# HorizonRobotics/HoloAgent

Hardware: AMD Instinct MI355X
Metric: HMSG frames/sec (one scene per GPU: map A1-A2, fusion A3-A5, merge A6, pooling A7, floors A8, rooms by the device watershed N1, room clouds, room embeddings and View nodes A9, objects with the view <-> object test A10 and graph assembly A11, nothing handed in -- plus 1000 coarse-to-fine retrieval qu (higher is better)
Workload: dtype f64 geometry / f32 features

## Files before the change

holoagent_amd/_lib.py:

```python
from __future__ import annotations

import ctypes as C
import os

import numpy as np

_HERE = os.path.dirname(os.path.abspath(__file__))
LIB_PATH = os.path.join(_HERE, "libhmsg.so")


class HmsgConfig(C.Structure):
    _fields_ = [
        ("device_id", C.c_int32), ("feat_dim", C.c_int32), ("height", C.c_int32), ("width", C.c_int32),
        ("max_frames", C.c_int32), ("max_masks", C.c_int32),
        ("voxel_size", C.c_double), ("depth_scale", C.c_double), ("init_overlap_thresh", C.c_double),
        ("overlap_thresh_factor", C.c_double), ("iou_thresh", C.c_double), ("clip_masked_weight", C.c_double),
        ("max_mask_distance", C.c_double), ("merge_type", C.c_int32), ("outlier_nb_points", C.c_int32),
        ("outlier_radius", C.c_double), ("pool_max_dist", C.c_double), ("feat_dbscan_eps", C.c_double),
        ("feat_dbscan_min", C.c_int32), ("merge_dbscan_eps", C.c_double), ("merge_dbscan_min", C.c_int32),
        ("min_instance_points", C.c_int32), ("skip_frames", C.c_int32), ("depth_cut", C.c_double), ("grid_resolution", C.c_double),
        ("overlap_distance_form", C.c_int32),
    ]


# ... 168 lines not shown
    "hmsg_test_allocator_carving": (C.c_int, [C.c_int32, C.c_int32]),
    "hmsg_test_dbscan": (C.c_int, [_P, C.c_int32, _P, C.c_double, C.c_int32, _P, _P, _P, _P, _P]),
    "hmsg_index_load_objects": (C.c_int, [C.c_int32, C.c_char_p, C.c_int64, _P, _P, C.c_int32, C.POINTER(_P), C.POINTER(C.c_int32)]),
    "hmsg_index_create": (C.c_int, [C.c_int32, C.c_int32, C.c_int64, _P, C.c_int32, _P, C.POINTER(_P)]),
    "hmsg_index_destroy": (None, [_P]),
    "hmsg_index_last_error": (C.c_char_p, [_P]),
    "hmsg_index_set_profiling": (C.c_int, [_P, C.c_int32]),
    "hmsg_index_profile": (C.c_int, [_P, C.POINTER(C.c_int64), C.POINTER(C.c_double), C.POINTER(C.c_double)]),
    "hmsg_query_objects": (C.c_int, [_P, C.c_int32, C.c_int32, _P, _P, _P, _P, C.c_int32, C.c_int32, _P, _P, _P]),
    "hmsg_similarity": (C.c_int, [_P, C.c_int32, _P, _P]),
    "hmsg_index_set_hierarchy": (C.c_int, [_P, C.c_int32, C.c_int32, _P, _P, _P, _P, _P, _P]),
    "hmsg_query_hier": (C.c_int, [_P, C.c_int32, C.c_int32, _P, _P, _P, _P, _P, C.c_int32, C.c_int32, C.c_int32, _P, _P, _P, _P, _P]),
    "hmsg_comm_unique_id": (C.c_int, [_P]),
    "hmsg_comm_create": (C.c_int, [_P, C.c_int32, C.c_int32, C.c_int32, C.POINTER(_P)]),
    "hmsg_comm_destroy": (None, [_P]),
    "hmsg_comm_last_error": (C.c_char_p, [_P]),
    "hmsg_allgather_nodes": (C.c_int, [_P, _P, C.c_int32, C.POINTER(_P), _P, _P]),
    "hmsg_allreduce_feature_sums": (C.c_int, [_P, _P]),
    "hmsg_test_sort_pairs": (C.c_int, [_P, _P, C.c_int64, C.c_int32]),
    "hmsg_test_repeat_add": (C.c_int, [_P, _P, _P, _P, C.c_int64]),
    "hmsg_test_ckdtree": (C.c_int, [_P, C.c_int64, _P, C.c_int64, _P, _P, _P]),
    "hmsg_test_boundary": (C.c_int, [C.c_int32, _P, C.c_int64]),
    "hmsg_test_group_pairs": (C.c_int, [C.c_int32, C.c_int64, _P, C.c_int32, _P, C.c_double, _P, C.c_int64, C.POINTER(C.c_int64)]),
    "hmsg_test_pool_rows": (C.c_int, [C.c_int32, C.c_int32, _P, _P, _P, _P, C.c_int64, C.c_int32, C.c_double, C.c_int32, _P]),
}
EXPORTED_SYMBOLS = tuple(_SIGS)


class HmsgLib:
    def __init__(self, path: str | None = None):
        path = path or LIB_PATH
        if not os.path.exists(path):
            raise HmsgError(
                f"{path} not found: build the HIP library first (python -c 'import __graft_entry__ as g; g.build()' "
                "or make -C holoagent_amd/csrc).  There is no CPU fallback.")
        self.path = path
        self.c = C.CDLL(path)
        for name, (res, args) in _SIGS.items():
            fn = getattr(self.c, name)
            fn.restype = res
            fn.argtypes = args
        if self.c.hmsg_config_size() != C.sizeof(HmsgConfig):
            raise HmsgError("struct hmsg_config of %s has %d bytes, the binding's HmsgConfig %d: rebuild the library or update "
                            "holoagent_amd/_lib.py" % (path, self.c.hmsg_config_size(), C.sizeof(HmsgConfig)))

    def default_config(self, **over) -> HmsgConfig:
# ... 1207 lines not shown
```

holoagent_amd/csrc/hmsg_merge.hip:

```cpp
#include "hmsg_boundary.h"
#include "hmsg_cloudops.h"
#include "hmsg_fold_host.h"

#include <algorithm>
#include <cmath>
#include <numeric>
#include <chrono>
#include <unordered_map>
#include <condition_variable>
#include <deque>
#include <mutex>
#include <thread>

namespace {

struct Cloud {
    long long off = 0;
    int n = 0;
    double mn[3] = {0, 0, 0}, mx[3] = {0, 0, 0};
    bool fixed = false;
    bool fresh = true;
    bool raw = false;
    bool anchor = false;
    unsigned long long uid = 0;
// ... 91 lines not shown
                           long long cursor_base, int chunk) {
    const OvGrid g = gr[find_entry(gr, ngr, blockIdx.x)];
    const int i0 = (int)(blockIdx.x - (unsigned)g.blk0) * chunk, i1 = min(g.n, i0 + chunk);
    for (int i = i0 + threadIdx.x; i < i1; i += blockDim.x) {
        const double* p = pool + (size_t)(g.pt_off + i) * 3;
        atomicAdd(&cursor[ov_cell(g, (float)p[0], (float)p[1], (float)p[2]) - cursor_base], 1u);
    }
}
__global__ void k_ov_fill(const double* __restrict__ pool, const OvGrid* __restrict__ gr, int ngr, const unsigned* __restrict__ cells,
                          unsigned* __restrict__ cursor, long long cursor_base, float* __restrict__ sorted, int chunk) {
    const OvGrid g = gr[find_entry(gr, ngr, blockIdx.x)];
    const int i0 = (int)(blockIdx.x - (unsigned)g.blk0) * chunk, i1 = min(g.n, i0 + chunk);
    for (int i = i0 + threadIdx.x; i < i1; i += blockDim.x) {
        const double* p = pool + (size_t)(g.pt_off + i) * 3;
        float x = (float)p[0], y = (float)p[1], z = (float)p[2];
        long long c = ov_cell(g, x, y, z);
        size_t pos = (size_t)g.ix_pt + cells[c] + (atomicSub(&cursor[c - cursor_base], 1u) - 1u);
        sorted[(size_t)pos * 3] = x;
        sorted[(size_t)pos * 3 + 1] = y;
        sorted[(size_t)pos * 3 + 2] = z;
    }
}

#define OV_UNROLL 4
__device__ __forceinline__ float ov_norm2(float a, float b, float c) { return __fadd_rn(__fadd_rn(__fmul_rn(a, a), __fmul_rn(b, b)), __fmul_rn(c, c)); }
template <bool BLAS>
__device__ __forceinline__ float ov_dist2(float x, float y, float z, float qx, float qy, float qz, float nx) {
    if (!BLAS) {
        const float ddx = __fsub_rn(x, qx), ddy = __fsub_rn(y, qy), ddz = __fsub_rn(z, qz);
        return __fadd_rn(__fadd_rn(__fmul_rn(ddx, ddx), __fmul_rn(ddy, ddy)), __fmul_rn(ddz, ddz));
    }
    const float ip = __fmaf_rn(z, qz, __fmaf_rn(y, qy, __fmul_rn(x, qx)));
    const float d = __fsub_rn(__fadd_rn(nx, ov_norm2(qx, qy, qz)), __fmul_rn(2.0f, ip));
    return d < 0.f ? 0.f : d;
}
template <bool BLAS = false>
__device__ __forceinline__ bool ov_scan(const float* __restrict__ sorted, unsigned s0, unsigned e0, float x, float y, float z,
                                        float r2, unsigned* ncand = nullptr, float nx = 0.f) {
    for (unsigned k = s0; k < e0; k += OV_UNROLL) {
        bool h = false;
#pragma unroll
        for (int j = 0; j < OV_UNROLL; ++j) {
            const unsigned kk = min(k + (unsigned)j, e0 - 1u);
            const float d2 = ov_dist2<BLAS>(x, y, z, sorted[(size_t)kk * 3], sorted[(size_t)kk * 3 + 1], sorted[(size_t)kk * 3 + 2], nx);
            h = h || (k + (unsigned)j < e0 && d2 < r2);
        }
// ... 376 lines not shown
            hipLaunchKernelGGL(k_gp_pairs<true>, dim3((unsigned)tiles.size()), dim3(GP_TILE), 0, s, d_box, d_tiles, iou_thresh, n,
                               (unsigned*)nullptr, (const unsigned*)start.p, h_out.p, cap);
            HMSG_CHECK_LAUNCH();
            spin.wait(s);
            const long long total = (long long)(unsigned)h_out.p[0];
            if (total <= cap) {
                *n_pairs = total;
                return h_out.p + 2;
            }
            cap_pairs = total;
            h_out.ensure(2 + 2 * (size_t)cap_pairs);
        }
    }
    static bool fits(const int* group_off, int n_groups) {
        unsigned long long worst = 0;
        for (int g = 0; g < n_groups; ++g) {
            const unsigned long long m = (unsigned long long)(group_off[g + 1] - group_off[g]);
            worst += m * (m ? m - 1 : 0) / 2;
        }
        return worst < (1ull << 32);
    }
};

double bbox_iou(const Cloud& a, const Cloud& b) {
    return box_iou(a.mn, a.mx, b.mn, b.mx);
}

struct IntSpan {
    const int* b;
    const int* e;
    size_t size() const { return (size_t)(e - b); }
    int operator[](size_t k) const { return b[k]; }
    const int* begin() const { return b; }
    const int* end() const { return e; }
};
struct CompList {
    std::vector<int> off, mem;
    size_t size() const { return off.empty() ? 0 : off.size() - 1; }
    IntSpan operator[](size_t c) const { return IntSpan{mem.data() + off[c], mem.data() + off[c + 1]}; }
};

struct Merger {
    hmsg_ctx* h = nullptr;
    hipStream_t s = nullptr;
    CloudOps ops;
    DevBuf<double> pool;
// ... 1 lines not shown
    long long pool_used = 0;
    DevBuf<unsigned> ix_cells;
    long long ix_cells_used = 0;
    DevBuf<float> ix_pts;
    long long ix_pts_used = 0;
    DevBuf<double> concat;
    DevBuf<unsigned char> concat_core;
    DevBuf<OvGrid> d_grids;
    PinnedBuf<OvGrid> h_grids;
    PinnedBuf<CatSeg> h_cat;
    DevBuf<unsigned> d_cursor;
    DevBuf<CatSeg> d_cat;
    DevBuf<unsigned long long> ovstat;
    Publisher pub_counts;
    PinnedBuf<char> h_ovpack;
    DevBuf<char> d_ovpack;
    PinnedBuf<OvSpec> h_spec[2];
    DevBuf<OvGrid> d_spec[2];
    int spec_turn = 0;
    std::vector<OvSpec> spec;
    std::vector<int> spec_of_seg;
    bool spec_wanted = getenv("HMSG_DEBUG_NO_SPEC_INDEX") == nullptr;
    double spec_built = 0, spec_built_pts = 0, spec_skipped = 0;
    size_t cursor_clean = 0;
    SpinWait spin;
    unsigned long long next_uid = 1;
    std::unordered_map<unsigned long long, double> ratio_cache;
    bool use_cache = false;
    bool use_anchor = true;
    bool inplace_wanted = getenv("HMSG_DEBUG_NO_INPLACE") == nullptr;
    double radius = 0;
    double reach = 0;
    int faiss_form = 0;
    double cell = 0;
    double eps = 0.1;
    int minpts = 10;
    double iou_thresh = 0.05;
    double tphase[6] = {0, 0, 0, 0, 0, 0};
    struct Stats {
        double steps = 0, clouds = 0, fresh_raw = 0, fresh_g = 0, pairs_raw = 0, pairs_g = 0;
        double scan1_raw = 0, scan2_raw = 0, scan1_g = 0, scan2_g = 0;
        double idx_pts = 0;
        double ccount[5] = {0, 0, 0, 0, 0}, cpts[5] = {0, 0, 0, 0, 0}, cB[5] = {0, 0, 0, 0, 0}, cmem[5] = {0, 0, 0, 0, 0};
        double cchanged[5] = {0, 0, 0, 0, 0}, cmulti[5] = {0, 0, 0, 0, 0}, ccontested[5] = {0, 0, 0, 0, 0}, cnonfixed[5] = {0, 0, 0, 0, 0};
    } st;
    bool want_stats = false;

    template <typename T>
    void grow(DevBuf<T>& b, size_t used_elems, size_t need_elems) {
        if (need_elems <= b.n) return;
        CarveScope carve;
        DevBuf<T> nb;
        nb.alloc(std::max(need_elems * 2, (size_t)1 << 18));
        if (used_elems) HIP_TRY(hipMemcpyAsync(nb.p, b.p, used_elems * sizeof(T), hipMemcpyDeviceToDevice, s));
        HIP_TRY(hipStreamSynchronize(s));
        nb.swap(b);
    }

    OvGrid grid_at(const Cloud& c, const float* lo, const int* gd, long long ix_cell, long long ix_pt, long long pt_off, int n) const {
        OvGrid g;
        g.blk0 = 0;
        g.next = -1;
        g.pt_off = pt_off;
        g.ix_cell = ix_cell;
        g.ix_pt = ix_pt;
        g.n = n;
        g.gx = gd[0];
        g.gy = gd[1];
        g.gz = gd[2];
        g.mnx = (float)c.mn[0]; g.mny = (float)c.mn[1]; g.mnz = (float)c.mn[2];
        g.mxx = (float)c.mx[0]; g.mxy = (float)c.mx[1]; g.mxz = (float)c.mx[2];
        g.ox = (double)lo[0] - 1e-3;
        g.oy = (double)lo[1] - 1e-3;
        g.oz = (double)lo[2] - 1e-3;
        g.cell = cell;
        return g;
    }
    void push_grids(const Cloud& c, std::vector<OvGrid>& g) const {
        g.push_back(grid_at(c, c.bmn, c.gd, c.ix_cell, c.ix_pt, c.off, c.n));
        g.back().blk0 = c.nb;
        if (c.has_delta) {
            g.back().next = (int)g.size();
            g.push_back(grid_at(c, c.dmn, c.gd2, c.ix_cell2, c.ix_pt2, c.off + c.nb, c.n - c.nb));
        }
    }

    void build_indices(std::vector<Cloud>& L) {
        std::vector<int> todo;
        long long ncell_new = 0, npts_new = 0;
        int maxn = 0;
        std::vector<OvGrid> g;
        unsigned nblk = 0;
        for (int i = 0; i < (int)L.size(); ++i) {
            Cloud& c = L[i];
            if (c.has_index || c.n == 0) continue;
            const float lo[3] = {(float)c.mn[0], (float)c.mn[1], (float)c.mn[2]};
            int gd[3];
            for (int a = 0; a < 3; ++a) gd[a] = (int)std::floor(((double)(float)c.mx[a] - (double)lo[a] + 2e-3) / cell) + 1;
            const long long ncell = (long long)gd[0] * gd[1] * gd[2] + 1;
// ... 165 lines not shown
                sp.delta_always = delta_always ? 1 : 0;
                sp.out_off = sd.out_mode ? sd.out_off : out_base;
                sp.ncell = ncell;
                spec_of_seg[(size_t)sg] = (int)spec.size();
                spec.push_back(sp);
                nblk += cdiv((size_t)sd.n, OVI_CHUNK);
                ncell_new += ncell;
                npts_max += sd.n;
            }
        if (spec.empty()) return;
        if (!(ncell_new < (1ll << 31) && npts_max < (1ll << 31))) {
            spec.clear();
            spec_of_seg.assign(segs.size(), -1);
            return;
        }
        grow(ix_cells, (size_t)ix_cells_used, (size_t)(ix_cells_used + ncell_new));
        grow(ix_pts, (size_t)ix_pts_used * 3, (size_t)(ix_pts_used + npts_max) * 3);
        spec_turn ^= 1;
        PinnedBuf<OvSpec>& hs = h_spec[spec_turn];
        DevBuf<OvGrid>& ds = d_spec[spec_turn];
        hs.ensure(spec.size());
        ds.ensure(spec.size());
        memcpy(hs.p, spec.data(), spec.size() * sizeof(OvSpec));
        hipLaunchKernelGGL(k_ov_spec, dim3(cdiv(spec.size(), 64)), dim3(64), 0, s, (const OvSpec*)hs.p, (int)spec.size(), d_res, K, ds.p);
        {
            const unsigned* before = d_cursor.p;
            d_cursor.ensure((size_t)ncell_new);
            if (d_cursor.p != before) cursor_clean = 0;
            if (cursor_clean < (size_t)ncell_new) {
                HIP_TRY(hipMemsetAsync(d_cursor.p, 0, d_cursor.n * 4, s));
                cursor_clean = d_cursor.n;
            }
        }
        hipLaunchKernelGGL(k_ov_count, dim3(nblk), dim3(256), 0, s, (const double*)pool.p, (const OvGrid*)ds.p, (int)spec.size(),
                           d_cursor.p, ix_cells_used, OVI_CHUNK);
        HMSG_CHECK_LAUNCH();
        hmsg_scan_u32(d_cursor.p, ix_cells.p + ix_cells_used, (size_t)ncell_new, s, ops.scan_tmp, nullptr);
        hipLaunchKernelGGL(k_ov_fill, dim3(nblk), dim3(256), 0, s, (const double*)pool.p, (const OvGrid*)ds.p, (int)spec.size(),
                           (const unsigned*)ix_cells.p, d_cursor.p, ix_cells_used, ix_pts.p, OVI_CHUNK);
        HMSG_CHECK_LAUNCH();
    }

    void overlap_ratios(const std::vector<Cloud>& L, const std::vector<std::pair<int, int>>& pairs, std::vector<double>& ratio,
                        double decide_th, std::vector<unsigned char>* second_ran = nullptr) {
        ratio.assign(pairs.size(), 0.0);
        if (second_ran) second_ran->assign(pairs.size(), 0);
        if (pairs.empty()) return;
        const size_t P = pairs.size();
        const auto pack_t0 = std::chrono::steady_clock::now();
        std::vector<int>& slot = ws_slot;
        std::vector<OvGrid>& g = ws_grids;
        std::vector<OvTask>& tasks = ws_tasks;
        slot.assign(L.size(), -1);
        g.clear();
        tasks.resize(P * 2);
        unsigned nblk1 = 0, nblk2 = 0;
        for (size_t k = 0; k < P; ++k) {
            int a = pairs[k].first, b = pairs[k].second;
            for (int v : {a, b})
                if (slot[v] < 0) {
                    slot[v] = (int)g.size();
                    push_grids(L[v], g);
                }
// ... 51 lines not shown
                if (nblk)
                    hipLaunchKernelGGL(ovk, dim3((unsigned)nblk), dim3(256), 0, s, (const double*)pool.p, dg, dt,
                                       (const unsigned*)ix_cells.p, (const float*)ix_pts.p, r2, r, (int)P, db, 0u, dc, (const unsigned*)nullptr, decide_th, OV_CHUNK,
                                       d_ovstat, ov_sorted_src, 0);
            } else {
                for (int dir = 0; dir < 2; ++dir) {
                    const unsigned nb = dir ? nblk2 : nblk1;
                    if (!nb) continue;
                    if (dir && plan) {
                        hipLaunchKernelGGL(ovk2, dim3(std::min(nb, 512u)), dim3(256), 0, s, (const double*)pool.p, dg, dt,
                                           (const unsigned*)ix_cells.p, (const float*)ix_pts.p, r2, r, (int)P, dc, decide_th, OV_CHUNK, d_ovstat, ov_sorted_src);
                        continue;
                    }
                    hipLaunchKernelGGL(ovk, dim3(nb + ((!dir && plan) ? (unsigned)P : 0u)), dim3(256), 0, s, (const double*)pool.p, dg, dt,
                                       (const unsigned*)ix_cells.p, (const float*)ix_pts.p, r2, r, (int)P, db, dir ? nblk1 : 0u, dc,
                                       (dir && decide_th >= 0.0) ? (const unsigned*)dc : (const unsigned*)nullptr, decide_th, OV_CHUNK, d_ovstat, ov_sorted_src,
                                       (!dir && plan) ? 1 : 0);
                }
            }
        }
        HMSG_CHECK_LAUNCH();
        pub_counts.launch(s, (const unsigned*)dc, tasks.size());
        pub_counts.wait();
        const unsigned* hc = pub_counts.data();
        double ov_work = 0;
        for (size_t k = 0; k < P; ++k) {
            const int na = std::min(L[pairs[k].first].n, L[pairs[k].second].n), nb = std::max(L[pairs[k].first].n, L[pairs[k].second].n);
            const bool bounded = (hc[P + k] & 0x80000000u) != 0;
            ratio[k] = std::max((double)hc[k] / (double)na, bounded ? 0.0 : (double)hc[P + k] / (double)nb);
            ov_work += 12.0 * ((double)na + (double)nb);
            if (!(decide_th >= 0.0 && (double)hc[k] / (double)na > decide_th) && !bounded) {
                if (second_ran) (*second_ran)[k] = 1;
            }
        }
        if (ops.prof->enabled && prof_idx < ops.prof->ev.size()) ops.prof->ev[prof_idx].work = ov_work;
    }

    void find_pairs(const std::vector<Cloud>& L, std::vector<std::pair<int, int>>& pairs, std::vector<double>& known,
                    std::vector<std::pair<int, int>>& known_pairs, const std::vector<int>* group_off = nullptr) {
        const int n = (int)L.size();
        auto candidate = [&](int i, int j) {
            if (use_cache && !L[i].fresh && !L[j].fresh) {
                auto it = ratio_cache.find(L[i].uid * 0x100000000ull + L[j].uid);
                if (it != ratio_cache.end()) {
                    known_pairs.emplace_back(i, j);
                    known.push_back(it->second);
// ... 289 lines not shown
            concat.ensure((size_t)cat_total * 3);
            concat_core.ensure((size_t)cat_total);
            grow(pool, (size_t)pool_used * 3, (size_t)(out_base + dense_total) * 3);
            grow(poolcore, (size_t)pool_used, (size_t)(out_base + dense_total));
            lap(3);
            DbGather ga;
            ga.pool = pool.p;
            ga.host_segs = cat.data();
            ga.nsegs = (int)cat.size();
            ga.poolcore = poolcore.p;
            ga.dstcore = use_anchor ? concat_core.p : nullptr;
            ga.pool_w = pool.p;
            ga.poolcore_w = poolcore.p;
            spec.clear();
            spec_of_seg.assign(segs.size(), -1);
            const bool speculate = spec_wanted && CloudOps::regions_supported();
            ops.dbscan_keep_largest(concat.p, segs, eps, minpts, pool.p + (size_t)out_base * 3, res,
                                    use_anchor ? (const unsigned char*)concat_core.p : nullptr, poolcore.p + out_base, &ga,
                                    (speculate || planned) ? std::function<void(const unsigned*, int)>([&](const unsigned* d_res, int K) {
                                        if (speculate) speculate_indices(L, comps, seg_of_comp, segs, out_base, d_res, K);
                                        advance_plan(true);
                                    }) : std::function<void(const unsigned*, int)>());
            advance_plan(false);
            lap(4);
            if (want_stats) {
                for (size_t c = 0; c < comps.size(); ++c) {
                    if (seg_of_comp[c] < 0) continue;
                    const auto& mem = comps[c];
                    const DbscanResult& r = res[seg_of_comp[c]];
                    long long tot = 0, rest = 0;
                    bool rest_raw = true;
                    for (size_t q = 0; q < mem.size(); ++q) {
                        tot += L[mem[q]].n;
                        if (q) {
                            rest += L[mem[q]].n;
                            rest_raw = rest_raw && L[mem[q]].raw;
                        }
                    }
                    int cls;
                    if (mem.size() == 1) cls = L[mem[0]].raw ? 0 : 1;
                    else if (L[mem[0]].anchor && L[mem[0]].n > rest) cls = rest_raw ? 2 : 3;
                    else cls = 4;
                    st.ccount[cls] += 1;
                    st.cpts[cls] += tot;
                    st.cB[cls] += mem.size() == 1 ? tot : rest;
                    st.cmem[cls] += mem.size();
// ... 262 lines not shown
    h->inst.off.assign(1, 0);
    h->inst.box.clear();
    for (auto& k : result) {
        if (k.n < min_points) continue;
        for (int a = 0; a < 3; ++a) h->inst.box.push_back(k.mn[a]);
        for (int a = 0; a < 3; ++a) h->inst.box.push_back(k.mx[a]);
        cat.push_back(CatSeg{k.off, keep_total, k.n, 0, (int)cat_blocks, 0});
        cat_blocks += cdiv((size_t)k.n, CAT_CHUNK);
        keep_total += k.n;
        h->inst.off.push_back(keep_total);
    }
    h->inst.total = keep_total;
    DevBuf<double> fresh;
    fresh.alloc((size_t)std::max<long long>(keep_total, 1) * 3);
    if (!cat.empty()) {
        m.d_cat.ensure(cat.size());
        HIP_TRY(hipMemcpyAsync(m.d_cat.p, cat.data(), cat.size() * sizeof(CatSeg), hipMemcpyHostToDevice, m.s));
        if (cat_blocks)
            hipLaunchKernelGGL(k_concat, dim3(cat_blocks), dim3(256), 0, m.s, (const double*)m.pool.p, (const CatSeg*)m.d_cat.p,
                               (int)cat.size(), fresh.p, (const unsigned char*)nullptr, (unsigned char*)nullptr, CAT_CHUNK);
        HMSG_CHECK_LAUNCH();
    }
    HIP_TRY(hipStreamSynchronize(m.s));
    fresh.swap(h->inst.pts);
}

double next_level_threshold(double th, double factor, long long lists) {
    return th - factor * (double)(lists - 2) / (double)std::max<long long>(1, lists - 1);
}

std::vector<std::vector<Cloud>> merge_level_batched(Merger& m, std::vector<std::vector<Cloud>>& lv, double th, long long max_points) {
    const long long bound = max_points < 0 ? 0x7fffffffll : max_points;
    std::vector<std::vector<Cloud>> nx;
    nx.reserve((lv.size() + 1) / 2);
    const size_t npairs = lv.size() / 2;
    std::vector<long long> pair_pts(npairs, 0), pair_clouds(npairs, 0);
    for (size_t k = 0; k < npairs; ++k)
        for (size_t q = 2 * k; q < 2 * k + 2; ++q) {
            pair_clouds[k] += (long long)lv[q].size();
            for (const Cloud& c : lv[q]) pair_pts[k] += c.n;
        }
    for (size_t k0 = 0; k0 < npairs;) {
        size_t k1 = k0;
        long long pts = 0, clouds = 0;
        do {
            pts += pair_pts[k1];
// ... 79 lines not shown
        const auto& t = m.st;
        const double S = std::max(1.0, t.steps);
        fprintf(stderr, "[mstat] steps %.0f  per step: clouds %.1f  fresh raw %.1f  fresh G %.1f  indexed pts %.0f\n", t.steps, t.clouds / S,
                t.fresh_raw / S, t.fresh_g / S, t.idx_pts / S);
        fprintf(stderr, "[mstat] pairs/step raw %.1f (scan1 %.0f scan2 %.0f pts)   G-fresh %.1f (scan1 %.0f scan2 %.0f pts)\n", t.pairs_raw / S,
                t.scan1_raw / S, t.scan2_raw / S, t.pairs_g / S, t.scan1_g / S, t.scan2_g / S);
        if (m.ovstat.p) {
            unsigned long long hs[16];
            (void)hipMemcpy(hs, m.ovstat.p, 128, hipMemcpyDeviceToHost);
            fprintf(stderr, "[mstat] overlap probes with > 32 candidates: %.1f per step, %.0f candidates per step; longest candidate list of a probe %llu\n",
                    hs[8] / S, hs[9] / S, hs[7]);
            fprintf(stderr, "[mstat] overlap probes/step %.0f: outside the box %.0f  hit own cell %.0f  hit neighbour %.0f  miss %.0f | candidates/step own %.0f  neighbour %.0f\n",
                    hs[0] / S, hs[1] / S, hs[2] / S, hs[3] / S, hs[4] / S, hs[5] / S, hs[6] / S);
        }
        const char* nmc[5] = {"singleton raw", "singleton non-fixed", "anchor+raw", "anchor+any", "other"};
        for (int c = 0; c < 5; ++c)
            fprintf(stderr, "[mstat] dbscan class %-20s comps/step %.2f  pts/step %.0f  B pts/step %.0f  members %.2f  changed %.0f multi %.0f contested %.0f nonfixed %.0f (totals)\n",
                    nmc[c], t.ccount[c] / S, t.cpts[c] / S, t.cB[c] / S, t.ccount[c] ? t.cmem[c] / t.ccount[c] : 0.0, t.cchanged[c],
                    t.cmulti[c], t.ccontested[c], t.cnonfixed[c]);
    }
    if (getenv("HMSG_DEBUG_TIMING"))
        fprintf(stderr, "[hmsg merge] overlap grids: %.0f over whole clouds (%.0f points), %.0f delta grids (%.0f points); of them behind the DBSCAN batches: %.0f (%.0f points), %.0f not needed\n", m.grid_full,
                m.grid_full_pts, m.grid_delta, m.grid_delta_pts, m.spec_built, m.spec_built_pts, m.spec_skipped);
    if (getenv("HMSG_DEBUG_TIMING") && (m.gp_device_batches > 0 || m.gp_host_batches > 0))
        fprintf(stderr, "[hmsg merge] level batches of several pairs: candidate pairs of %.0f listed on the device (k_gp_pairs; inside 'pairs(host)' above), of %.0f by the host's loop\n",
                m.gp_device_batches, m.gp_host_batches);
    if (getenv("HMSG_DEBUG_TIMING") && m.n_collects)
        fprintf(stderr, "[hmsg merge] %d collections of the point pool / grid arenas\n", m.n_collects);
    if (getenv("HMSG_DEBUG_TIMING") && m.ops.stat_calls > 0)
        fprintf(stderr, "[hmsg merge] dbscan batches %.0f: mean points %.0f  grid cells %.0f  occupied cells %.0f  counted points %.0f\n",
                m.ops.stat_calls, m.ops.stat_points / m.ops.stat_calls, m.ops.stat_cells / m.ops.stat_calls,
                m.ops.stat_core_cells / m.ops.stat_calls, m.ops.stat_needy / m.ops.stat_calls);
    if (getenv("HMSG_DEBUG_TIMING") && m.ops.stat_calls > 0)
        fprintf(stderr, "[hmsg merge] dbscan segments with a cropped anchor member: %.0f (%.0f anchor points a batch), %.0f of them in place; pool %.2f GB\n",
                m.ops.stat_forced, m.ops.stat_forced_first / m.ops.stat_calls, m.ops.stat_inplace, (double)m.pool_used * 24 / 1e9);
    if (getenv("HMSG_DEBUG_MAXCELL") && m.ops.stat_calls > 0)
        fprintf(stderr, "[hmsg merge] fullest cell of a dbscan batch: mean %.0f points, max %.0f\n", m.ops.stat_maxcell_sum / m.ops.stat_calls, m.ops.stat_maxcell_max);
}

struct SeqFold {
    Folder m;
    hmsg_ctx* h = nullptr;
    std::vector<std::vector<Cloud>> frames;
    size_t f_next = 0;
    size_t prebuilt_upto = 0;
    std::vector<Cloud> G;
// ... 370 lines not shown
    m.ops.bounds(m.pool.p, segs);
    std::vector<Cloud> L;
    for (auto& sd : segs) {
        if (sd.n == 0) continue;
        Cloud k;
        k.off = sd.pt_base;
        k.n = sd.n;
        k.uid = m.next_uid++;
        for (int a = 0; a < 3; ++a) {
            k.mn[a] = sd.mn[a];
            k.mx[a] = sd.mx[a];
        }
        L.push_back(k);
    }
    std::vector<Cloud> result = n_ext > 0 ? m.merge_3d_masks(std::move(L), th) : std::move(L);
    if (final_pass) result = m.merge_3d_masks(std::move(result), 0.75);
    store_instances(m, h, result, final_pass ? c.min_instance_points : 0);
    if (final_pass) {
        h->merged = true;
        h->tree_partial = false;
    }
}

extern "C" int hmsg_test_group_pairs(int32_t device_id, int64_t n, const double* boxes, int32_t n_groups, const int64_t* group_off,
                                     double iou_thresh, int32_t* pairs_out, int64_t capacity, int64_t* n_pairs) {
    if (n < 0 || n > 0x7fffffffll || n_groups < 0 || !group_off || !n_pairs || capacity < 0 || (n > 0 && !boxes) || (capacity > 0 && !pairs_out))
        return HMSG_ERR_INVALID;
    *n_pairs = 0;
    return hmsg_boundary("hmsg_test_group_pairs", device_id, [&] {
        std::vector<int> off((size_t)n_groups + 1);
        for (int g = 0; g <= n_groups; ++g) {
            HMSG_REQUIRE(group_off[g] >= (g ? group_off[g - 1] : 0) && group_off[g] <= n, HMSG_ERR_INVALID, "group_off must ascend from 0 to n");
            off[(size_t)g] = (int)group_off[g];
        }
        HMSG_REQUIRE(off[0] == 0 && off[(size_t)n_groups] == (int)n, HMSG_ERR_INVALID, "group_off must ascend from 0 to n");
        HMSG_REQUIRE(GroupPairs::fits(off.data(), n_groups), HMSG_ERR_UNSUPPORTED, "the groups hold 2^32 pairs or more");
        ScopedStream s(hipStreamNonBlocking);
        {
            GroupPairs gp;
            DevBuf<unsigned> scan_tmp;
            long long np = 0;
            const int* pr = gp.run(s, scan_tmp, nullptr, boxes, (int)n, off.data(), n_groups, iou_thresh, &np);
            *n_pairs = np;
            const long long m = std::min<long long>(np, capacity);
            if (m) memcpy(pairs_out, pr, (size_t)m * 8);
        }
// ... 260 lines not shown
```

Before: 2731.

## Fuse overlap-grid spec, count, scan and fill into fewer kernel launches

Adds k_ov_build, which carries the grid spec entries as kernel arguments so the separate k_ov_spec launch and its host-to-device copy are no longer needed, and folds spec decoding into the count kernel. The default path (form 3) uses three launches: fused spec+count, scan, fill. An opt-in single-launch form has count, decoupled-lookback scan and fill workgroups coordinate through device counters with polling and an error flag. The aim is to cut launch and copy overhead for the many small grid builds behind the DBSCAN batches. The single-launch form depends on all workgroups making progress and can fail on a timeout, so it stays behind an environment variable and the legacy path is kept as a fallback.

```diff
diff --git a/holoagent_amd/_lib.py b/holoagent_amd/_lib.py
--- a/holoagent_amd/_lib.py
+++ b/holoagent_amd/_lib.py
@@ -214,6 +214,8 @@
     "hmsg_test_ckdtree": (C.c_int, [_P, C.c_int64, _P, C.c_int64, _P, _P, _P]),
     "hmsg_test_boundary": (C.c_int, [C.c_int32, _P, C.c_int64]),
     "hmsg_test_group_pairs": (C.c_int, [C.c_int32, C.c_int64, _P, C.c_int32, _P, C.c_double, _P, C.c_int64, C.POINTER(C.c_int64)]),
+    "hmsg_test_ov_build": (C.c_int, [C.c_int32, C.c_int32, _P, C.c_int64, C.c_int32, _P, _P, _P, C.c_double, _P, C.c_int64, C.c_int32, C.c_int64,
+                                     C.c_int64, C.c_int64, _P, _P, _P, _P, _P, _P, _P]),
     "hmsg_test_pool_rows": (C.c_int, [C.c_int32, C.c_int32, _P, _P, _P, _P, C.c_int64, C.c_int32, C.c_double, C.c_int32, _P]),
 }
 EXPORTED_SYMBOLS = tuple(_SIGS)
diff --git a/holoagent_amd/csrc/hmsg_merge.hip b/holoagent_amd/csrc/hmsg_merge.hip
--- a/holoagent_amd/csrc/hmsg_merge.hip
+++ b/holoagent_amd/csrc/hmsg_merge.hip
@@ -137,6 +137,250 @@
     }
 }
 
+static const int OVB_MAX_SPECS = 36;
+static const unsigned OVB_MAX_POLLS = 1u << 19;
+struct OvbEntry {
+    int blk0, seg, n_in, nb_first, n_first;
+    int flags;
+    long long out_off, ix_cell;
+    int gd[3];
+    double o[3];
+    float box[6];
+};
+struct OvBuildArgs {
+    const double* pool;
+    const unsigned* res;
+    OvGrid* table;
+    unsigned* cursor;
+    unsigned* cells;
+    float* sorted;
+    unsigned long long* scan_state;
+    unsigned* sync;
+    unsigned* err;
+    long long cursor_base, ix_pt;
+    double cell;
+    int K, nspec;
+    unsigned ncell, nblk, ntile, epoch, count_target, scan_target;
+    OvbEntry ent[OVB_MAX_SPECS];
+};
+static OvbEntry ovb_entry(const OvSpec& sp) {
+    OvbEntry e;
+    e.blk0 = sp.g.blk0;
+    e.seg = sp.seg;
+    e.n_in = sp.n_in;
+    e.nb_first = sp.nb_first;
+    e.n_first = sp.n_first;
+    e.flags = (sp.singleton ? 1 : 0) | (sp.inherit ? 2 : 0) | (sp.delta_always ? 4 : 0) | (sp.out_mode << 4);
+    e.out_off = sp.out_off;
+    e.ix_cell = sp.g.ix_cell;
+    e.gd[0] = sp.g.gx; e.gd[1] = sp.g.gy; e.gd[2] = sp.g.gz;
+    e.o[0] = sp.g.ox; e.o[1] = sp.g.oy; e.o[2] = sp.g.oz;
+    e.box[0] = sp.g.mnx; e.box[1] = sp.g.mny; e.box[2] = sp.g.mnz;
+    e.box[3] = sp.g.mxx; e.box[4] = sp.g.mxy; e.box[5] = sp.g.mxz;
+    return e;
+}
+__device__ __forceinline__ OvGrid ovb_grid(const OvBuildArgs& a, unsigned wb, int* entry) {
+    int e = 0, hi = a.nspec - 1;
+    while (e < hi) {
+        const int mid = (e + hi + 1) >> 1;
+        if ((unsigned)a.ent[mid].blk0 <= wb) e = mid; else hi = mid - 1;
+    }
+    *entry = e;
+    const OvbEntry& en = a.ent[e];
+    OvSpec sp;
+    sp.seg = en.seg;
+    sp.singleton = en.flags & 1;
+    sp.inherit = (en.flags >> 1) & 1;
+    sp.delta_always = (en.flags >> 2) & 1;
+    sp.out_mode = en.flags >> 4;
+    sp.nb_first = en.nb_first;
+    sp.n_first = en.n_first;
+    sp.n_in = en.n_in;
+    sp.out_off = en.out_off;
+    sp.ncell = (long long)en.gd[0] * en.gd[1] * en.gd[2] + 1;
+    int n_out, first_kept, start, first, n_idx;
+    ov_spec_result(sp, a.res, a.K, &n_out, &first_kept, &start);
+    ov_spec_decide(sp, n_out, first_kept, &first, &n_idx);
+    OvGrid g;
+    g.blk0 = en.blk0;
+    g.next = -1;
+    g.pt_off = sp.out_off + (sp.out_mode == 0 ? (long long)start : 0ll) + first;
+    g.ix_pt = a.ix_pt;
+    g.ix_cell = en.ix_cell;
+    g.n = n_idx;
+    g.gx = en.gd[0]; g.gy = en.gd[1]; g.gz = en.gd[2];
+    g.mnx = en.box[0]; g.mny = en.box[1]; g.mnz = en.box[2];
+    g.mxx = en.box[3]; g.mxy = en.box[4]; g.mxz = en.box[5];
+    g.ox = en.o[0];
+    g.oy = en.o[1];
+    g.oz = en.o[2];
+    g.cell = a.cell;
+    return g;
+}
+__device__ __forceinline__ void ovb_drain() {
+#ifndef HMSG_EMU_BUILD
+    asm volatile("s_waitcnt vmcnt(0)" ::: "memory");
+#endif
+}
+__device__ __forceinline__ void ovb_pause() {
+#ifndef HMSG_EMU_BUILD
+    __builtin_amdgcn_s_sleep(8);
+#endif
+}
+__device__ __forceinline__ void ovb_fail(unsigned* err, unsigned code) {
+    __hip_atomic_store(err, code, __ATOMIC_RELAXED, __HIP_MEMORY_SCOPE_SYSTEM);
+}
+__device__ __forceinline__ bool ovb_wait(unsigned* ctr, unsigned target, unsigned* err, unsigned code) {
+    for (unsigned polls = 0;; ++polls) {
+        const unsigned v = __hip_atomic_load(ctr, __ATOMIC_RELAXED, __HIP_MEMORY_SCOPE_AGENT);
+        if ((int)(v - target) >= 0) return true;
+        if (polls >= OVB_MAX_POLLS) {
+            ovb_fail(err, code);
+            return false;
+        }
+        ovb_pause();
+    }
+}
+__device__ __forceinline__ unsigned ovb_lookback_prefix(unsigned long long* __restrict__ state, long long tile, unsigned epoch, unsigned agg,
+                                                        bool* ok) {
+    const int lane = threadIdx.x & 63;
+    *ok = true;
+    if (lane == 0)
+        __hip_atomic_store(&state[tile], scan_pack(epoch, tile == 0 ? 2u : 1u, agg), __ATOMIC_RELAXED, __HIP_MEMORY_SCOPE_AGENT);
+    unsigned prefix = 0;
+    if (tile > 0) {
+        long long hi = tile - 1;
+        for (unsigned polls = 0;;) {
+            const long long idx = hi - lane;
+            unsigned long long sw = scan_pack(epoch, 2u, 0u);
+            if (idx >= 0) sw = __hip_atomic_load(&state[idx], __ATOMIC_RELAXED, __HIP_MEMORY_SCOPE_AGENT);
+            const unsigned tag = (unsigned)(sw >> 32);
+            const unsigned flag = (tag >> 2) == (epoch & 0x3fffffffu) ? (tag & 3u) : 0u;
+            const unsigned long long has_prefix = __ballot(flag == 2u), not_ready = __ballot(flag == 0u);
+            unsigned long long take = ~0ull;
+            if (has_prefix) {
+                const int first = __ffsll(has_prefix) - 1;
+                take = first == 63 ? ~0ull : ((1ull << (first + 1)) - 1ull);
+            }
+            if (not_ready & take) {
+                if (++polls > OVB_MAX_POLLS) {
+                    *ok = false;
+                    return 0;
+                }
+                ovb_pause();
+                continue;
+            }
+            unsigned part = ((take >> lane) & 1ull) ? (unsigned)sw : 0u;
+            for (int o = 32; o > 0; o >>= 1) part += __shfl_xor(part, o);
+            prefix += part;
+            if (has_prefix) break;
+            hi -= 64;
+        }
+        if (lane == 0)
+            __hip_atomic_store(&state[tile], scan_pack(epoch, 2u, prefix + agg), __ATOMIC_RELAXED, __HIP_MEMORY_SCOPE_AGENT);
+    }
+    return prefix;
+}
+template <bool ONE>
+__global__ void __launch_bounds__(256) k_ov_build(const OvBuildArgs a) {
+    __shared__ unsigned s_wsum[4];
+    __shared__ unsigned s_prefix;
+    __shared__ int s_ok;
+    const int tid = threadIdx.x;
+    const unsigned b = blockIdx.x;
+    if (ONE && b >= a.nblk && b < a.nblk + a.ntile) {
+        if (tid == 0) s_ok = ovb_wait(&a.sync[0], a.count_target, a.err, 1u) ? 1 : 0;
+        __syncthreads();
+        if (!s_ok) return;
+        const int lane = tid & 63, w = tid >> 6;
+        const long long tile = (long long)(b - a.nblk);
+        const size_t base = ((size_t)tile * 256 + tid) * 4;
+        unsigned v[4];
+        unsigned t = 0;
+        for (int i = 0; i < 4; ++i) {
+            v[i] = base + i < a.ncell ? __hip_atomic_load(&a.cursor[base + i], __ATOMIC_RELAXED, __HIP_MEMORY_SCOPE_AGENT) : 0u;
+            t += v[i];
+        }
+        unsigned incl = t;
+        for (int o = 1; o < 64; o <<= 1) {
+            unsigned u = __shfl_up(incl, o);
+            if (lane >= o) incl += u;
+        }
+        if (lane == 63) s_wsum[w] = incl;
+        __syncthreads();
+        unsigned woff = 0;
+        for (int i = 0; i < w; ++i) woff += s_wsum[i];
+        const unsigned agg = s_wsum[0] + s_wsum[1] + s_wsum[2] + s_wsum[3];
+        if (w == 0) {
+            bool ok;
+            const unsigned prefix = ovb_lookback_prefix(a.scan_state, tile, a.epoch, agg, &ok);
+            if (lane == 0) {
+                s_prefix = prefix;
+                s_ok = ok ? 1 : 0;
+                if (!ok) ovb_fail(a.err, 3u);
+            }
+        }
+        __syncthreads();
+        if (!s_ok) return;
+        unsigned excl = s_prefix + woff + incl - t;
+        for (int i = 0; i < 4; ++i) {
+            if (base + i < a.ncell) __hip_atomic_store(&a.cells[base + i], excl, __ATOMIC_RELAXED, __HIP_MEMORY_SCOPE_AGENT);
+            excl += v[i];
+        }
+        ovb_drain();
+        __syncthreads();
+        if (tid == 0) atomicAdd(&a.sync[32], 1u);
+        return;
+    }
+    const bool fill = ONE && b >= a.nblk;
+    const unsigned wb = fill ? b - a.nblk - a.ntile : b;
+    int e;
+    const OvGrid g = ovb_grid(a, wb, &e);
+    const int i0 = (int)(wb - (unsigned)g.blk0) * OVI_CHUNK, i1 = min(g.n, i0 + OVI_CHUNK);
+    if (!fill) {
+        if (wb == (unsigned)g.blk0 && tid == 0) {
+            static_assert(sizeof(OvGrid) % 8 == 0, "OvGrid is stored in 8-byte words");
+            unsigned long long w[sizeof(OvGrid) / 8];
+            memcpy(w, &g, sizeof(OvGrid));
+            for (size_t i = 0; i < sizeof(OvGrid) / 8; ++i)
+                __hip_atomic_store(reinterpret_cast<unsigned long long*>(&a.table[e]) + i, w[i], __ATOMIC_RELAXED, __HIP_MEMORY_SCOPE_AGENT);
+        }
+        for (int i = i0 + tid; i < i1; i += 256) {
+            const double* p = a.pool + (size_t)(g.pt_off + i) * 3;
+            atomicAdd(&a.cursor[ov_cell(g, (float)p[0], (float)p[1], (float)p[2]) - a.cursor_base], 1u);
+        }
+        if (!ONE) return;
+        ovb_drain();
+        __syncthreads();
+        if (tid == 0) atomicAdd(&a.sync[0], 1u);
+        return;
+    }
+    constexpr int PER = OVI_CHUNK / 256;
+    float x[PER], y[PER], z[PER];
+    long long c[PER];
+    for (int k = 0; k < PER; ++k) {
+        const int i = i0 + tid + k * 256;
+        c[k] = -1;
+        if (i < i1) {
+            const double* p = a.pool + (size_t)(g.pt_off + i) * 3;
+            x[k] = (float)p[0];
+            y[k] = (float)p[1];
+            z[k] = (float)p[2];
+            c[k] = ov_cell(g, x[k], y[k], z[k]) - a.cursor_base;
+        }
+    }
+    if (tid == 0) s_ok = ovb_wait(&a.sync[32], a.scan_target, a.err, 2u) ? 1 : 0;
+    __syncthreads();
+    if (!s_ok) return;
+    for (int k = 0; k < PER; ++k) {
+        if (c[k] < 0) continue;
+        const unsigned start = __hip_atomic_load(&a.cells[c[k]], __ATOMIC_RELAXED, __HIP_MEMORY_SCOPE_AGENT);
+        const size_t pos = (size_t)g.ix_pt + start + (atomicSub(&a.cursor[c[k]], 1u) - 1u);
+        a.sorted[pos * 3] = x[k];
+        a.sorted[pos * 3 + 1] = y[k];
+        a.sorted[pos * 3 + 2] = z[k];
+    }
+}
 #define OV_UNROLL 4
 __device__ __forceinline__ float ov_norm2(float a, float b, float c) { return __fadd_rn(__fadd_rn(__fmul_rn(a, a), __fmul_rn(b, b)), __fmul_rn(c, c)); }
 template <bool BLAS>
@@ -559,6 +803,112 @@
     }
 };
 
+static OvGrid ov_grid_at(const double* mn, const double* mx, const float* lo, const int* gd, long long ix_cell, long long ix_pt, long long pt_off,
+                         int n, double cell) {
+    OvGrid g;
+    g.blk0 = 0;
+    g.next = -1;
+    g.pt_off = pt_off;
+    g.ix_cell = ix_cell;
+    g.ix_pt = ix_pt;
+    g.n = n;
+    g.gx = gd[0];
+    g.gy = gd[1];
+    g.gz = gd[2];
+    g.mnx = (float)mn[0]; g.mny = (float)mn[1]; g.mnz = (float)mn[2];
+    g.mxx = (float)mx[0]; g.mxy = (float)mx[1]; g.mxz = (float)mx[2];
+    g.ox = (double)lo[0] - 1e-3;
+    g.oy = (double)lo[1] - 1e-3;
+    g.oz = (double)lo[2] - 1e-3;
+    g.cell = cell;
+    return g;
+}
+
+struct OvBuilder {
+    DevBuf<unsigned> sync;
+    PinnedBuf<unsigned> err;
+    unsigned count_total = 0, scan_total = 0;
+    double n_one = 0, n_three = 0, n_legacy = 0, cells_one = 0, blocks_one = 0, specs_one = 0;
+
+    static bool fits(int form, size_t nspec, long long ncell, long long max_cells) {
+        return nspec <= (size_t)OVB_MAX_SPECS && ncell < (1ll << 31) && (form != 1 || ncell <= max_cells);
+    }
+    void legacy(hipStream_t s, const double* pool, const OvSpec* hs, int nspec, const unsigned* d_res, int K, OvGrid* table, unsigned nblk,
+                unsigned* cursor, long long cursor_base, long long ncell, unsigned* ix_cells, float* ix_pts, DevBuf<unsigned>& scan_tmp) {
+        hipLaunchKernelGGL(k_ov_spec, dim3(cdiv((size_t)nspec, 64)), dim3(64), 0, s, hs, nspec, d_res, K, table);
+        hipLaunchKernelGGL(k_ov_count, dim3(nblk), dim3(256), 0, s, pool, (const OvGrid*)table, nspec, cursor, cursor_base, OVI_CHUNK);
+        HMSG_CHECK_LAUNCH();
+        hmsg_scan_u32(cursor, ix_cells + cursor_base, (size_t)ncell, s, scan_tmp, nullptr);
+        hipLaunchKernelGGL(k_ov_fill, dim3(nblk), dim3(256), 0, s, pool, (const OvGrid*)table, nspec, (const unsigned*)ix_cells, cursor,
+                           cursor_base, ix_pts, OVI_CHUNK);
+        HMSG_CHECK_LAUNCH();
+        n_legacy += 1;
+    }
+    void build(int form, hipStream_t s, const double* pool, const std::vector<OvSpec>& spec, const unsigned* d_res, int K, OvGrid* table,
+               unsigned nblk, unsigned* cursor, long long cursor_base, long long ncell, unsigned* ix_cells, float* ix_pts, double cell,
+               DevBuf<unsigned>& scan_tmp) {
+        static_assert(sizeof(OvBuildArgs) <= 4096, "k_ov_build's arguments exceed what a launch carries");
+        OvBuildArgs a;
+        a.pool = pool;
+        a.res = d_res;
+        a.table = table;
+        a.cursor = cursor;
+        a.cells = ix_cells + cursor_base;
+        a.sorted = ix_pts;
+        a.cursor_base = cursor_base;
+        a.ix_pt = spec[0].g.ix_pt;
+        a.cell = cell;
+        a.K = K;
+        a.nspec = (int)spec.size();
+        a.ncell = (unsigned)ncell;
+        a.nblk = nblk;
+        for (size_t j = 0; j < spec.size(); ++j) a.ent[j] = ovb_entry(spec[j]);
+        if (form == 3) {
+            a.ntile = 0;
+            a.scan_state = nullptr;
+            a.sync = a.err = nullptr;
+            a.epoch = a.count_target = a.scan_target = 0;
+            hipLaunchKernelGGL(k_ov_build<false>, dim3(nblk), dim3(256), 0, s, a);
+            HMSG_CHECK_LAUNCH();
+            hmsg_scan_u32(cursor, ix_cells + cursor_base, (size_t)ncell, s, scan_tmp, nullptr);
+            hipLaunchKernelGGL(k_ov_fill, dim3(nblk), dim3(256), 0, s, pool, (const OvGrid*)table, (int)spec.size(), (const unsigned*)ix_cells,
+                               cursor, cursor_base, ix_pts, OVI_CHUNK);
+            HMSG_CHECK_LAUNCH();
+            n_three += 1;
+            return;
+        }
+        if (!sync.p) {
+            sync.alloc(64);
+            HIP_TRY(hipMemsetAsync(sync.p, 0, 64 * 4, s));
+            err.ensure(4);
+            err.p[0] = 0;
+            count_total = scan_total = 0;
+        }
+        a.ntile = (unsigned)cdiv((size_t)ncell, 1024);
+        a.epoch = hmsg_scan_epoch(scan_tmp, a.ntile, s);
+        a.scan_state = reinterpret_cast<unsigned long long*>(scan_tmp.p);
+        a.sync = sync.p;
+        a.count_target = (count_total += nblk);
+        a.scan_target = (scan_total += a.ntile);
+        a.err = err.p;
+        hipLaunchKernelGGL(k_ov_build<true>, dim3(2 * nblk + a.ntile), dim3(256), 0, s, a);
+        HMSG_CHECK_LAUNCH();
+        n_one += 1;
+        cells_one += (double)ncell;
+        blocks_one += 2.0 * nblk + a.ntile;
+        specs_one += (double)spec.size();
+    }
+    void check() {
+        if (!err.p) return;
+        const unsigned code = *(volatile unsigned*)err.p;
+        if (!code) return;
+        err.p[0] = 0;
+        sync.release();
+        throw hmsg_error{HMSG_ERR_HIP, std::string("k_ov_build: a workgroup gave up waiting for ") +
+                                           (code == 1 ? "the count roles" : code == 2 ? "the scan roles" : "a scan tile's predecessors")};
+    }
+};
+
 double bbox_iou(const Cloud& a, const Cloud& b) {
     return box_iou(a.mn, a.mx, b.mn, b.mx);
 }
@@ -606,6 +956,11 @@
     std::vector<int> spec_of_seg;
     bool spec_wanted = getenv("HMSG_DEBUG_NO_SPEC_INDEX") == nullptr;
     double spec_built = 0, spec_built_pts = 0, spec_skipped = 0;
+    OvBuilder ovb;
+    int ov_build_form = (getenv("HMSG_OV_BUILD_LEGACY") && atoi(getenv("HMSG_OV_BUILD_LEGACY")) == 1)           ? 0
+                        : (getenv("HMSG_OV_BUILD_ONE_LAUNCH") && atoi(getenv("HMSG_OV_BUILD_ONE_LAUNCH")) == 1) ? 1
+                                                                                                                : 3;
+    long long ov_build_max_cells = getenv("HMSG_DEBUG_OV_BUILD_MAX_CELLS") ? atoll(getenv("HMSG_DEBUG_OV_BUILD_MAX_CELLS")) : (1ll << 20);
     size_t cursor_clean = 0;
     SpinWait spin;
     unsigned long long next_uid = 1;
@@ -642,23 +997,7 @@
     }
 
     OvGrid grid_at(const Cloud& c, const float* lo, const int* gd, long long ix_cell, long long ix_pt, long long pt_off, int n) const {
-        OvGrid g;
-        g.blk0 = 0;
-        g.next = -1;
-        g.pt_off = pt_off;
-        g.ix_cell = ix_cell;
-        g.ix_pt = ix_pt;
-        g.n = n;
-        g.gx = gd[0];
-        g.gy = gd[1];
-        g.gz = gd[2];
-        g.mnx = (float)c.mn[0]; g.mny = (float)c.mn[1]; g.mnz = (float)c.mn[2];
-        g.mxx = (float)c.mx[0]; g.mxy = (float)c.mx[1]; g.mxz = (float)c.mx[2];
-        g.ox = (double)lo[0] - 1e-3;
-        g.oy = (double)lo[1] - 1e-3;
-        g.oz = (double)lo[2] - 1e-3;
-        g.cell = cell;
-        return g;
+        return ov_grid_at(c.mn, c.mx, lo, gd, ix_cell, ix_pt, pt_off, n, cell);
     }
     void push_grids(const Cloud& c, std::vector<OvGrid>& g) const {
         g.push_back(grid_at(c, c.bmn, c.gd, c.ix_cell, c.ix_pt, c.off, c.n));
@@ -870,7 +1209,6 @@
         hs.ensure(spec.size());
         ds.ensure(spec.size());
         memcpy(hs.p, spec.data(), spec.size() * sizeof(OvSpec));
-        hipLaunchKernelGGL(k_ov_spec, dim3(cdiv(spec.size(), 64)), dim3(64), 0, s, (const OvSpec*)hs.p, (int)spec.size(), d_res, K, ds.p);
         {
             const unsigned* before = d_cursor.p;
             d_cursor.ensure((size_t)ncell_new);
@@ -880,13 +1218,12 @@
                 cursor_clean = d_cursor.n;
             }
         }
-        hipLaunchKernelGGL(k_ov_count, dim3(nblk), dim3(256), 0, s, (const double*)pool.p, (const OvGrid*)ds.p, (int)spec.size(),
-                           d_cursor.p, ix_cells_used, OVI_CHUNK);
-        HMSG_CHECK_LAUNCH();
-        hmsg_scan_u32(d_cursor.p, ix_cells.p + ix_cells_used, (size_t)ncell_new, s, ops.scan_tmp, nullptr);
-        hipLaunchKernelGGL(k_ov_fill, dim3(nblk), dim3(256), 0, s, (const double*)pool.p, (const OvGrid*)ds.p, (int)spec.size(),
-                           (const unsigned*)ix_cells.p, d_cursor.p, ix_cells_used, ix_pts.p, OVI_CHUNK);
-        HMSG_CHECK_LAUNCH();
+        if (ov_build_form && OvBuilder::fits(ov_build_form, spec.size(), ncell_new, ov_build_max_cells))
+            ovb.build(ov_build_form, s, pool.p, spec, d_res, K, ds.p, nblk, d_cursor.p, ix_cells_used, ncell_new, ix_cells.p, ix_pts.p, cell,
+                      ops.scan_tmp);
+        else
+            ovb.legacy(s, pool.p, hs.p, (int)spec.size(), d_res, K, ds.p, nblk, d_cursor.p, ix_cells_used, ncell_new, ix_cells.p, ix_pts.p,
+                       ops.scan_tmp);
     }
 
     void overlap_ratios(const std::vector<Cloud>& L, const std::vector<std::pair<int, int>>& pairs, std::vector<double>& ratio,
@@ -984,6 +1321,7 @@
         HMSG_CHECK_LAUNCH();
         pub_counts.launch(s, (const unsigned*)dc, tasks.size());
         pub_counts.wait();
+        ovb.check();
         const unsigned* hc = pub_counts.data();
         double ov_work = 0;
         for (size_t k = 0; k < P; ++k) {
@@ -1319,6 +1657,7 @@
                                         advance_plan(true);
                                     }) : std::function<void(const unsigned*, int)>());
             advance_plan(false);
+            ovb.check();
             lap(4);
             if (want_stats) {
                 for (size_t c = 0; c < comps.size(); ++c) {
@@ -1627,6 +1966,7 @@
         HMSG_CHECK_LAUNCH();
     }
     HIP_TRY(hipStreamSynchronize(m.s));
+    m.ovb.check();
     fresh.swap(h->inst.pts);
 }
 
@@ -1752,6 +2092,10 @@
     if (getenv("HMSG_DEBUG_TIMING"))
         fprintf(stderr, "[hmsg merge] overlap grids: %.0f over whole clouds (%.0f points), %.0f delta grids (%.0f points); of them behind the DBSCAN batches: %.0f (%.0f points), %.0f not needed\n", m.grid_full,
                 m.grid_full_pts, m.grid_delta, m.grid_delta_pts, m.spec_built, m.spec_built_pts, m.spec_skipped);
+    if (getenv("HMSG_DEBUG_TIMING"))
+        fprintf(stderr, "[hmsg merge] grid builds behind the DBSCAN batches: %.0f in three launches (entries as kernel arguments), %.0f in one launch (k_ov_build: %.1f grids, %.0f cells, %.0f workgroups a launch), %.0f by the four legacy launches\n",
+                m.ovb.n_three, m.ovb.n_one, m.ovb.n_one ? m.ovb.specs_one / m.ovb.n_one : 0.0, m.ovb.n_one ? m.ovb.cells_one / m.ovb.n_one : 0.0,
+                m.ovb.n_one ? m.ovb.blocks_one / m.ovb.n_one : 0.0, m.ovb.n_legacy);
     if (getenv("HMSG_DEBUG_TIMING") && (m.gp_device_batches > 0 || m.gp_host_batches > 0))
         fprintf(stderr, "[hmsg merge] level batches of several pairs: candidate pairs of %.0f listed on the device (k_gp_pairs; inside 'pairs(host)' above), of %.0f by the host's loop\n",
                 m.gp_device_batches, m.gp_host_batches);
@@ -2168,6 +2512,98 @@
     }
 }
 
+extern "C" int hmsg_test_ov_build(int32_t device_id, int32_t new_form, const double* pts, int64_t n_pts, int32_t n_spec, const int32_t* spec_i,
+                                  const int64_t* spec_off, const double* spec_box, double cell, const uint32_t* res, int64_t n_res, int32_t K,
+                                  int64_t max_cells, int64_t cell_cap, int64_t pt_cap, int64_t* layout, int64_t* totals, uint32_t* cells_out,
+                                  float* sorted_out, uint32_t* cursor_out, uint8_t* grids_out, int32_t* one_launch_out) {
+    if ((new_form != 1 && new_form != 3) || n_pts <= 0 || n_pts > 0x7fffffffll || !pts || n_spec <= 0 || !spec_i || !spec_off || !spec_box || !(cell > 0) || !res || K <= 0 ||
+        n_res < (int64_t)K * 18 + 8 || cell_cap <= 0 || pt_cap <= 0 || !layout || !totals || !cells_out || !sorted_out || !cursor_out ||
+        !grids_out || !one_launch_out)
+        return HMSG_ERR_INVALID;
+    return hmsg_boundary("hmsg_test_ov_build", device_id, [&] {
+        const long long cells_used = 37, pts_used = 11;
+        std::vector<OvSpec> spec((size_t)n_spec);
+        long long ncell_new = 0, npts_max = 0, pts_idx = 0;
+        unsigned nblk = 0;
+        for (int j = 0; j < n_spec; ++j) {
+            const int32_t* si = spec_i + (size_t)j * 8;
+            const double* bx = spec_box + (size_t)j * 6;
+            HMSG_REQUIRE(si[0] >= 0 && si[0] < K && si[5] > 0 && si[6] >= 0 && si[6] <= 2, HMSG_ERR_INVALID, "hmsg_test_ov_build: bad spec entry");
+            const float lo[3] = {(float)bx[0], (float)bx[1], (float)bx[2]};
+            int gd[3];
+            for (int a = 0; a < 3; ++a) {
+                HMSG_REQUIRE(bx[3 + a] >= bx[a], HMSG_ERR_INVALID, "hmsg_test_ov_build: empty box");
+                gd[a] = (int)std::floor(((double)(float)bx[3 + a] - (double)lo[a] + 2e-3) / cell) + 1;
+            }
+            const long long ncell = (long long)gd[0] * gd[1] * gd[2] + 1;
+            OvSpec& sp = spec[(size_t)j];
+            sp.g = ov_grid_at(bx, bx + 3, lo, gd, cells_used + ncell_new, pts_used, 0, 0, cell);
+            sp.g.blk0 = (int)nblk;
+            sp.seg = si[0];
+            sp.singleton = si[1];
+            sp.inherit = si[2];
+            sp.nb_first = si[3];
+            sp.n_first = si[4];
+            sp.n_in = si[5];
+            sp.out_mode = si[6];
+            sp.delta_always = si[7];
+            sp.out_off = spec_off[j];
+            sp.ncell = ncell;
+            int n_out, first_kept, start, first, n_idx;
+            ov_spec_result(sp, res, K, &n_out, &first_kept, &start);
+            ov_spec_decide(sp, n_out, first_kept, &first, &n_idx);
+            const long long p0 = sp.out_off + (sp.out_mode == 0 ? (long long)start : 0ll) + first;
+            HMSG_REQUIRE(n_idx >= 0 && n_idx <= sp.n_in && p0 >= 0 && p0 + n_idx <= n_pts, HMSG_ERR_INVALID,
+                         "hmsg_test_ov_build: a grid's points lie outside the point array");
+            layout[(size_t)j * 2] = ncell_new;
+            layout[(size_t)j * 2 + 1] = ncell;
+            nblk += cdiv((size_t)sp.n_in, OVI_CHUNK);
+            ncell_new += ncell;
+            npts_max += sp.n_in;
+            pts_idx += n_idx;
+        }
+        totals[0] = ncell_new;
+        totals[1] = pts_idx;
+        totals[2] = (long long)sizeof(OvGrid);
+        HMSG_REQUIRE(ncell_new <= cell_cap && npts_max <= pt_cap && ncell_new < (1ll << 31), HMSG_ERR_INVALID, "hmsg_test_ov_build: capacities too small");
+        ScopedStream s(hipStreamNonBlocking);
+        DevBuf<double> pool;
+        DevBuf<unsigned> d_res, ix_cells, cursor, scan_tmp;
+        DevBuf<float> ix_pts;
+        DevBuf<OvGrid> table;
+        PinnedBuf<OvSpec> hs;
+        OvBuilder ovb;
+        pool.alloc((size_t)n_pts * 3);
+        d_res.alloc((size_t)n_res);
+        ix_cells.alloc((size_t)(cells_used + ncell_new));
+        cursor.alloc((size_t)ncell_new);
+        ix_pts.alloc((size_t)(pts_used + npts_max) * 3);
+        table.alloc((size_t)n_spec);
+        hs.ensure((size_t)n_spec);
+        memcpy(hs.p, spec.data(), spec.size() * sizeof(OvSpec));
+        HIP_TRY(hipMemcpyAsync(pool.p, pts, (size_t)n_pts * 24, hipMemcpyHostToDevice, s));
+        HIP_TRY(hipMemcpyAsync(d_res.p, res, (size_t)n_res * 4, hipMemcpyHostToDevice, s));
+        HIP_TRY(hipMemsetAsync(cursor.p, 0, (size_t)ncell_new * 4, s));
+        for (int form = 0; form < 2; ++form) {
+            HIP_TRY(hipMemsetAsync(ix_cells.p, 0xff, ix_cells.bytes(), s));
+            HIP_TRY(hipMemsetAsync(ix_pts.p, 0xff, ix_pts.bytes(), s));
+            HIP_TRY(hipMemsetAsync(table.p, 0xff, table.bytes(), s));
+            const bool one = form == 1 && OvBuilder::fits(new_form, spec.size(), ncell_new, max_cells);
+            if (form == 1) *one_launch_out = one ? 1 : 0;
+            if (one)
+                ovb.build(new_form, s, pool.p, spec, d_res.p, K, table.p, nblk, cursor.p, cells_used, ncell_new, ix_cells.p, ix_pts.p, cell, scan_tmp);
+            else
+                ovb.legacy(s, pool.p, hs.p, n_spec, d_res.p, K, table.p, nblk, cursor.p, cells_used, ncell_new, ix_cells.p, ix_pts.p, scan_tmp);
+            HIP_TRY(hipStreamSynchronize(s));
+            ovb.check();
+            HIP_TRY(hipMemcpy(cells_out + (size_t)form * cell_cap, ix_cells.p + cells_used, (size_t)ncell_new * 4, hipMemcpyDeviceToHost));
+            HIP_TRY(hipMemcpy(cursor_out + (size_t)form * cell_cap, cursor.p, (size_t)ncell_new * 4, hipMemcpyDeviceToHost));
+            HIP_TRY(hipMemcpy(sorted_out + (size_t)form * pt_cap * 3, ix_pts.p + (size_t)pts_used * 3, (size_t)npts_max * 12, hipMemcpyDeviceToHost));
+            HIP_TRY(hipMemcpy(grids_out + (size_t)form * n_spec * sizeof(OvGrid), table.p, (size_t)n_spec * sizeof(OvGrid), hipMemcpyDeviceToHost));
+        }
+    });
+}
+
 extern "C" int hmsg_test_group_pairs(int32_t device_id, int64_t n, const double* boxes, int32_t n_groups, const int64_t* group_off,
                                      double iou_thresh, int32_t* pairs_out, int64_t capacity, int64_t* n_pairs) {
     if (n < 0 || n > 0x7fffffffll || n_groups < 0 || !group_off || !n_pairs || capacity < 0 || (n > 0 && !boxes) || (capacity > 0 && !pairs_out))
```

New measurement: 2752, median of 6. No clear change (+0.8%).
